# reazon-research/ReazonSpeech

Hardware: NVIDIA H100
Metric: RTFx (audio-s/wall-s) FastConformer-RNNT 619M (higher is better)
Workload: dtype bf16

## Files before the change

reazonspeech_b200/csrc/common.cuh:

```cuda
#pragma once
#include <cuda_bf16.h>
#include <cuda_fp16.h>
#include <cuda_runtime.h>
#include <stdint.h>

#include <atomic>

namespace rs {

struct DeviceOnce {
  std::atomic<unsigned long long> done{0};
  bool pending() const { int d = 0; cudaGetDevice(&d); return ((done.load(std::memory_order_acquire) >> (d & 63)) & 1ull) == 0; }
  void set() { int d = 0; cudaGetDevice(&d); done.fetch_or(1ull << (d & 63), std::memory_order_release); }
};

constexpr int kWarp = 32;

__device__ __forceinline__ uint32_t smem_u32(const void* p) {
  return static_cast<uint32_t>(__cvta_generic_to_shared(p));
}
__device__ __forceinline__ int lane_id() { return threadIdx.x & 31; }
__device__ __forceinline__ int warp_id_uniform() { return __shfl_sync(0xffffffffu, threadIdx.x >> 5, 0); }

__device__ __forceinline__ float warp_sum(float v) {
#pragma unroll
  for (int o = 16; o > 0; o >>= 1) v += __shfl_xor_sync(0xffffffffu, v, o);
  return v;
}
__device__ __forceinline__ float warp_max(float v) {
#pragma unroll
  for (int o = 16; o > 0; o >>= 1) v = fmaxf(v, __shfl_xor_sync(0xffffffffu, v, o));
  return v;
}

__device__ __forceinline__ uint32_t pack_bf16x2(float lo, float hi) {
  __nv_bfloat162 t = __floats2bfloat162_rn(lo, hi);
  return *reinterpret_cast<uint32_t*>(&t);
}
__device__ __forceinline__ uint32_t pack_f16x2(float lo, float hi) {
  __half2 t = __floats2half2_rn(lo, hi);
  return *reinterpret_cast<uint32_t*>(&t);
}
__device__ __forceinline__ float2 unpack_bf16x2(uint32_t v) {
  __nv_bfloat162 t = *reinterpret_cast<__nv_bfloat162*>(&v);
  return __bfloat1622float2(t);
}
__device__ __forceinline__ float bf16_lo(uint32_t v) { return __uint_as_float(v << 16); }
__device__ __forceinline__ float bf16_hi(uint32_t v) { return __uint_as_float(v & 0xffff0000u); }

__device__ __forceinline__ float sigmoidf_fast(float x) {
  float e, r;
  asm("ex2.approx.ftz.f32 %0, %1;" : "=f"(e) : "f"(x * -1.4426950408889634f));
  asm("rcp.approx.ftz.f32 %0, %1;" : "=f"(r) : "f"(1.0f + e));
  return r;
}
__device__ __forceinline__ float sigmoidf_accurate(float x) { return 1.0f / (1.0f + expf(-x)); }
__device__ __forceinline__ float swishf_fast(float x) { return x * sigmoidf_fast(x); }

__device__ __forceinline__ void mbar_init(uint32_t bar, uint32_t count) {
  asm volatile("mbarrier.init.shared::cta.b64 [%0], %1;" ::"r"(bar), "r"(count));
}
__device__ __forceinline__ void fence_barrier_init() {
  asm volatile("fence.mbarrier_init.release.cluster;" ::: "memory");
}
__device__ __forceinline__ void fence_proxy_async() {
  asm volatile("fence.proxy.async.shared::cta;" ::: "memory");
}
__device__ __forceinline__ void mbar_arrive(uint32_t bar) {
  asm volatile("mbarrier.arrive.shared::cta.b64 _, [%0];" ::"r"(bar) : "memory");
}
__device__ __forceinline__ void mbar_arrive_expect_tx(uint32_t bar, uint32_t bytes) {
  asm volatile("mbarrier.arrive.expect_tx.shared::cta.b64 _, [%0], %1;" ::"r"(bar), "r"(bytes) : "memory");
}
__device__ __forceinline__ bool mbar_try_wait(uint32_t bar, uint32_t parity) {
  uint32_t ok;
  asm volatile(
      "{\n\t.reg .pred p;\n\t"
      "mbarrier.try_wait.parity.shared::cta.b64 p, [%1], %2;\n\t"
      "selp.u32 %0, 1, 0, p;\n\t}"
      : "=r"(ok)
      : "r"(bar), "r"(parity)
      : "memory");
  return ok != 0;
}
__device__ __forceinline__ void mbar_wait(uint32_t bar, uint32_t parity) {
  while (!mbar_try_wait(bar, parity)) {
  }
}

__device__ __forceinline__ void tma_prefetch_desc(const void* desc) {
  asm volatile("prefetch.tensormap [%0];" ::"l"(desc) : "memory");
}
__device__ __forceinline__ void tma_load_2d(uint32_t smem_dst, const void* desc, int c0, int c1, uint32_t bar) {
  asm volatile(
      "cp.async.bulk.tensor.2d.shared::cluster.global.tile.mbarrier::complete_tx::bytes [%0], [%1, {%3, %4}], [%2];"
      ::"r"(smem_dst), "l"(desc), "r"(bar), "r"(c0), "r"(c1)
      : "memory");
}

__device__ __forceinline__ void tma_store_2d(const void* desc, uint32_t smem_src, int c0, int c1) {
  asm volatile("cp.async.bulk.tensor.2d.global.shared::cta.bulk_group [%0, {%2, %3}], [%1];"
               ::"l"(desc), "r"(smem_src), "r"(c0), "r"(c1) : "memory");
}
__device__ __forceinline__ void tma_reduce_add_2d(const void* desc, uint32_t smem_src, int c0, int c1) {
  asm volatile("cp.reduce.async.bulk.tensor.2d.global.shared::cta.add.tile.bulk_group [%0, {%2, %3}], [%1];"
               ::"l"(desc), "r"(smem_src), "r"(c0), "r"(c1) : "memory");
}
__device__ __forceinline__ void bulk_commit() { asm volatile("cp.async.bulk.commit_group;" ::: "memory"); }
template <int N>
__device__ __forceinline__ void bulk_wait_read() { asm volatile("cp.async.bulk.wait_group.read %0;" ::"n"(N) : "memory"); }
template <int N>
__device__ __forceinline__ void bulk_wait() { asm volatile("cp.async.bulk.wait_group %0;" ::"n"(N) : "memory"); }

__device__ __forceinline__ void cp_async16(void* smem, const void* gmem) {
  asm volatile("cp.async.cg.shared.global [%0], [%1], 16;" ::"r"(smem_u32(smem)), "l"(gmem) : "memory");
}
__device__ __forceinline__ void cp_async_wait_all() { asm volatile("cp.async.wait_all;" ::: "memory"); }

__device__ __forceinline__ void stmatrix_x4(uint32_t addr, uint32_t r0, uint32_t r1, uint32_t r2, uint32_t r3) {
  asm volatile("stmatrix.sync.aligned.m8n8.x4.shared.b16 [%0], {%1, %2, %3, %4};"
               ::"r"(addr), "r"(r0), "r"(r1), "r"(r2), "r"(r3) : "memory");
}
__device__ __forceinline__ void stmatrix_x4_trans(uint32_t addr, uint32_t r0, uint32_t r1, uint32_t r2, uint32_t r3) {
  asm volatile("stmatrix.sync.aligned.m8n8.x4.trans.shared.b16 [%0], {%1, %2, %3, %4};"
               ::"r"(addr), "r"(r0), "r"(r1), "r"(r2), "r"(r3) : "memory");
}

template <int N>
__device__ __forceinline__ void setmaxnreg_dec() { asm volatile("setmaxnreg.dec.sync.aligned.u32 %0;" ::"n"(N)); }
template <int N>
__device__ __forceinline__ void setmaxnreg_inc() { asm volatile("setmaxnreg.inc.sync.aligned.u32 %0;" ::"n"(N)); }

__device__ __forceinline__ void wgmma_fence() { asm volatile("wgmma.fence.sync.aligned;" ::: "memory"); }
__device__ __forceinline__ void wgmma_commit() { asm volatile("wgmma.commit_group.sync.aligned;" ::: "memory"); }
template <int N>
__device__ __forceinline__ void wgmma_wait() { asm volatile("wgmma.wait_group.sync.aligned %0;" ::"n"(N) : "memory"); }
__device__ __forceinline__ void named_bar_sync(int id, int threads) { asm volatile("bar.sync %0, %1;" ::"r"(id), "r"(threads) : "memory"); }

__device__ __forceinline__ uint64_t wgmma_desc_k_sw128(uint32_t smem_addr) {
  uint64_t d = 0;
  d |= static_cast<uint64_t>((smem_addr & 0x3ffffu) >> 4);
  d |= static_cast<uint64_t>(1) << 16;
  d |= static_cast<uint64_t>(1024 >> 4) << 32;
  d |= static_cast<uint64_t>(1) << 62;
  return d;
}

__device__ __forceinline__ void wgmma_bf16_ss_n32(float (&d)[16], uint64_t desc_a, uint64_t desc_b, uint32_t accumulate) {
  asm volatile(
      "{\n\t.reg .pred p;\n\t"
      "setp.ne.b32 p, %18, 0;\n\t"
      "wgmma.mma_async.sync.aligned.m64n32k16.f32.bf16.bf16 "
      "{%0, %1, %2, %3, %4, %5, %6, %7, %8, %9, %10, %11, %12, %13, %14, %15}, %16, %17, p, 1, 1, 0, 0;\n\t}"
      :
        "+f"(d[0]), "+f"(d[1]), "+f"(d[2]), "+f"(d[3]), "+f"(d[4]), "+f"(d[5]), "+f"(d[6]), "+f"(d[7]),
        "+f"(d[8]), "+f"(d[9]), "+f"(d[10]), "+f"(d[11]), "+f"(d[12]), "+f"(d[13]), "+f"(d[14]), "+f"(d[15])
      : "l"(desc_a), "l"(desc_b), "r"(accumulate));
}

__device__ __forceinline__ void wgmma_bf16_ss_n64(float (&d)[32], uint64_t desc_a, uint64_t desc_b, uint32_t accumulate) {
  asm volatile(
      "{\n\t.reg .pred p;\n\t"
      "setp.ne.b32 p, %34, 0;\n\t"
      "wgmma.mma_async.sync.aligned.m64n64k16.f32.bf16.bf16 "
      "{%0, %1, %2, %3, %4, %5, %6, %7, %8, %9, %10, %11, %12, %13, %14, %15, %16, %17, %18, %19, %20, %21, %22, %23, %24, %25, %26, %27, %28, %29, %30, %31}, %32, %33, p, 1, 1, 0, 0;\n\t}"
      :
        "+f"(d[0]), "+f"(d[1]), "+f"(d[2]), "+f"(d[3]), "+f"(d[4]), "+f"(d[5]), "+f"(d[6]), "+f"(d[7]),
        "+f"(d[8]), "+f"(d[9]), "+f"(d[10]), "+f"(d[11]), "+f"(d[12]), "+f"(d[13]), "+f"(d[14]), "+f"(d[15]),
        "+f"(d[16]), "+f"(d[17]), "+f"(d[18]), "+f"(d[19]), "+f"(d[20]), "+f"(d[21]), "+f"(d[22]), "+f"(d[23]),
        "+f"(d[24]), "+f"(d[25]), "+f"(d[26]), "+f"(d[27]), "+f"(d[28]), "+f"(d[29]), "+f"(d[30]), "+f"(d[31])
      : "l"(desc_a), "l"(desc_b), "r"(accumulate));
}

__device__ __forceinline__ void wgmma_bf16_ss_n128(float (&d)[64], uint64_t desc_a, uint64_t desc_b, uint32_t accumulate) {
  asm volatile(
      "{\n\t.reg .pred p;\n\t"
      "setp.ne.b32 p, %66, 0;\n\t"
      "wgmma.mma_async.sync.aligned.m64n128k16.f32.bf16.bf16 "
      "{%0, %1, %2, %3, %4, %5, %6, %7, %8, %9, %10, %11, %12, %13, %14, %15, %16, %17, %18, %19, %20, %21, %22, %23, %24, %25, %26, %27, %28, %29, %30, %31, %32, %33, %34, %35, %36, %37, %38, %39, %40, %41, %42, %43, %44, %45, %46, %47, %48, %49, %50, %51, %52, %53, %54, %55, %56, %57, %58, %59, %60, %61, %62, %63}, %64, %65, p, 1, 1, 0, 0;\n\t}"
      :
        "+f"(d[0]), "+f"(d[1]), "+f"(d[2]), "+f"(d[3]), "+f"(d[4]), "+f"(d[5]), "+f"(d[6]), "+f"(d[7]),
        "+f"(d[8]), "+f"(d[9]), "+f"(d[10]), "+f"(d[11]), "+f"(d[12]), "+f"(d[13]), "+f"(d[14]), "+f"(d[15]),
        "+f"(d[16]), "+f"(d[17]), "+f"(d[18]), "+f"(d[19]), "+f"(d[20]), "+f"(d[21]), "+f"(d[22]), "+f"(d[23]),
        "+f"(d[24]), "+f"(d[25]), "+f"(d[26]), "+f"(d[27]), "+f"(d[28]), "+f"(d[29]), "+f"(d[30]), "+f"(d[31]),
        "+f"(d[32]), "+f"(d[33]), "+f"(d[34]), "+f"(d[35]), "+f"(d[36]), "+f"(d[37]), "+f"(d[38]), "+f"(d[39]),
        "+f"(d[40]), "+f"(d[41]), "+f"(d[42]), "+f"(d[43]), "+f"(d[44]), "+f"(d[45]), "+f"(d[46]), "+f"(d[47]),
        "+f"(d[48]), "+f"(d[49]), "+f"(d[50]), "+f"(d[51]), "+f"(d[52]), "+f"(d[53]), "+f"(d[54]), "+f"(d[55]),
        "+f"(d[56]), "+f"(d[57]), "+f"(d[58]), "+f"(d[59]), "+f"(d[60]), "+f"(d[61]), "+f"(d[62]), "+f"(d[63])
      : "l"(desc_a), "l"(desc_b), "r"(accumulate));
}

__device__ __forceinline__ void wgmma_bf16_ss_n256(float (&d)[128], uint64_t desc_a, uint64_t desc_b, uint32_t accumulate) {
  asm volatile(
      "{\n\t.reg .pred p;\n\t"
      "setp.ne.b32 p, %130, 0;\n\t"
      "wgmma.mma_async.sync.aligned.m64n256k16.f32.bf16.bf16 "
      "{%0, %1, %2, %3, %4, %5, %6, %7, %8, %9, %10, %11, %12, %13, %14, %15, %16, %17, %18, %19, %20, %21, %22, %23, %24, %25, %26, %27, %28, %29, %30, %31, "
      "%32, %33, %34, %35, %36, %37, %38, %39, %40, %41, %42, %43, %44, %45, %46, %47, %48, %49, %50, %51, %52, %53, %54, %55, %56, %57, %58, %59, %60, %61, %62, %63, "
      "%64, %65, %66, %67, %68, %69, %70, %71, %72, %73, %74, %75, %76, %77, %78, %79, %80, %81, %82, %83, %84, %85, %86, %87, %88, %89, %90, %91, %92, %93, %94, %95, "
      "%96, %97, %98, %99, %100, %101, %102, %103, %104, %105, %106, %107, %108, %109, %110, %111, %112, %113, %114, %115, %116, %117, %118, %119, %120, %121, %122, %123, %124, %125, %126, %127}, "
      "%128, %129, p, 1, 1, 0, 0;\n\t}"
      :
        "+f"(d[0]), "+f"(d[1]), "+f"(d[2]), "+f"(d[3]), "+f"(d[4]), "+f"(d[5]), "+f"(d[6]), "+f"(d[7]),
        "+f"(d[8]), "+f"(d[9]), "+f"(d[10]), "+f"(d[11]), "+f"(d[12]), "+f"(d[13]), "+f"(d[14]), "+f"(d[15]),
        "+f"(d[16]), "+f"(d[17]), "+f"(d[18]), "+f"(d[19]), "+f"(d[20]), "+f"(d[21]), "+f"(d[22]), "+f"(d[23]),
        "+f"(d[24]), "+f"(d[25]), "+f"(d[26]), "+f"(d[27]), "+f"(d[28]), "+f"(d[29]), "+f"(d[30]), "+f"(d[31]),
        "+f"(d[32]), "+f"(d[33]), "+f"(d[34]), "+f"(d[35]), "+f"(d[36]), "+f"(d[37]), "+f"(d[38]), "+f"(d[39]),
        "+f"(d[40]), "+f"(d[41]), "+f"(d[42]), "+f"(d[43]), "+f"(d[44]), "+f"(d[45]), "+f"(d[46]), "+f"(d[47]),
        "+f"(d[48]), "+f"(d[49]), "+f"(d[50]), "+f"(d[51]), "+f"(d[52]), "+f"(d[53]), "+f"(d[54]), "+f"(d[55]),
        "+f"(d[56]), "+f"(d[57]), "+f"(d[58]), "+f"(d[59]), "+f"(d[60]), "+f"(d[61]), "+f"(d[62]), "+f"(d[63]),
        "+f"(d[64]), "+f"(d[65]), "+f"(d[66]), "+f"(d[67]), "+f"(d[68]), "+f"(d[69]), "+f"(d[70]), "+f"(d[71]),
        "+f"(d[72]), "+f"(d[73]), "+f"(d[74]), "+f"(d[75]), "+f"(d[76]), "+f"(d[77]), "+f"(d[78]), "+f"(d[79]),
        "+f"(d[80]), "+f"(d[81]), "+f"(d[82]), "+f"(d[83]), "+f"(d[84]), "+f"(d[85]), "+f"(d[86]), "+f"(d[87]),
        "+f"(d[88]), "+f"(d[89]), "+f"(d[90]), "+f"(d[91]), "+f"(d[92]), "+f"(d[93]), "+f"(d[94]), "+f"(d[95]),
        "+f"(d[96]), "+f"(d[97]), "+f"(d[98]), "+f"(d[99]), "+f"(d[100]), "+f"(d[101]), "+f"(d[102]), "+f"(d[103]),
        "+f"(d[104]), "+f"(d[105]), "+f"(d[106]), "+f"(d[107]), "+f"(d[108]), "+f"(d[109]), "+f"(d[110]), "+f"(d[111]),
        "+f"(d[112]), "+f"(d[113]), "+f"(d[114]), "+f"(d[115]), "+f"(d[116]), "+f"(d[117]), "+f"(d[118]), "+f"(d[119]),
        "+f"(d[120]), "+f"(d[121]), "+f"(d[122]), "+f"(d[123]), "+f"(d[124]), "+f"(d[125]), "+f"(d[126]), "+f"(d[127])
      : "l"(desc_a), "l"(desc_b), "r"(accumulate));
}

__device__ __forceinline__ void wgmma_f16_ss_n64(float (&d)[32], uint64_t desc_a, uint64_t desc_b, uint32_t accumulate) {
  asm volatile(
      "{\n\t.reg .pred p;\n\t"
      "setp.ne.b32 p, %34, 0;\n\t"
      "wgmma.mma_async.sync.aligned.m64n64k16.f32.f16.f16 "
      "{%0, %1, %2, %3, %4, %5, %6, %7, %8, %9, %10, %11, %12, %13, %14, %15, %16, %17, %18, %19, %20, %21, %22, %23, %24, %25, %26, %27, %28, %29, %30, %31}, %32, %33, p, 1, 1, 0, 0;\n\t}"
      :
        "+f"(d[0]), "+f"(d[1]), "+f"(d[2]), "+f"(d[3]), "+f"(d[4]), "+f"(d[5]), "+f"(d[6]), "+f"(d[7]),
        "+f"(d[8]), "+f"(d[9]), "+f"(d[10]), "+f"(d[11]), "+f"(d[12]), "+f"(d[13]), "+f"(d[14]), "+f"(d[15]),
        "+f"(d[16]), "+f"(d[17]), "+f"(d[18]), "+f"(d[19]), "+f"(d[20]), "+f"(d[21]), "+f"(d[22]), "+f"(d[23]),
        "+f"(d[24]), "+f"(d[25]), "+f"(d[26]), "+f"(d[27]), "+f"(d[28]), "+f"(d[29]), "+f"(d[30]), "+f"(d[31])
      : "l"(desc_a), "l"(desc_b), "r"(accumulate));
}

__device__ __forceinline__ void wgmma_bf16_rs_n128(float (&d)[64], const uint32_t (&a)[4], uint64_t desc_b, uint32_t accumulate) {
  asm volatile(
      "{\n\t.reg .pred p;\n\t"
      "setp.ne.b32 p, %69, 0;\n\t"
      "wgmma.mma_async.sync.aligned.m64n128k16.f32.bf16.bf16 "
      "{%0, %1, %2, %3, %4, %5, %6, %7, %8, %9, %10, %11, %12, %13, %14, %15, %16, %17, %18, %19, %20, %21, %22, %23, %24, %25, %26, %27, %28, %29, %30, %31, %32, %33, %34, %35, %36, %37, %38, %39, %40, %41, %42, %43, %44, %45, %46, %47, %48, %49, %50, %51, %52, %53, %54, %55, %56, %57, %58, %59, %60, %61, %62, %63}, {%64, %65, %66, %67}, %68, p, 1, 1, 0;\n\t}"
      :
        "+f"(d[0]), "+f"(d[1]), "+f"(d[2]), "+f"(d[3]), "+f"(d[4]), "+f"(d[5]), "+f"(d[6]), "+f"(d[7]),
        "+f"(d[8]), "+f"(d[9]), "+f"(d[10]), "+f"(d[11]), "+f"(d[12]), "+f"(d[13]), "+f"(d[14]), "+f"(d[15]),
        "+f"(d[16]), "+f"(d[17]), "+f"(d[18]), "+f"(d[19]), "+f"(d[20]), "+f"(d[21]), "+f"(d[22]), "+f"(d[23]),
        "+f"(d[24]), "+f"(d[25]), "+f"(d[26]), "+f"(d[27]), "+f"(d[28]), "+f"(d[29]), "+f"(d[30]), "+f"(d[31]),
        "+f"(d[32]), "+f"(d[33]), "+f"(d[34]), "+f"(d[35]), "+f"(d[36]), "+f"(d[37]), "+f"(d[38]), "+f"(d[39]),
        "+f"(d[40]), "+f"(d[41]), "+f"(d[42]), "+f"(d[43]), "+f"(d[44]), "+f"(d[45]), "+f"(d[46]), "+f"(d[47]),
        "+f"(d[48]), "+f"(d[49]), "+f"(d[50]), "+f"(d[51]), "+f"(d[52]), "+f"(d[53]), "+f"(d[54]), "+f"(d[55]),
        "+f"(d[56]), "+f"(d[57]), "+f"(d[58]), "+f"(d[59]), "+f"(d[60]), "+f"(d[61]), "+f"(d[62]), "+f"(d[63])
      : "r"(a[0]), "r"(a[1]), "r"(a[2]), "r"(a[3]), "l"(desc_b), "r"(accumulate));
}


__device__ __forceinline__ uint4 ldg_nc_v4(const void* p) {
  uint4 r;
  asm volatile("ld.global.nc.L1::no_allocate.v4.u32 {%0, %1, %2, %3}, [%4];" : "=r"(r.x), "=r"(r.y), "=r"(r.z), "=r"(r.w) : "l"(p));
  return r;
}

}
```

reazonspeech_b200/csrc/gemm_wgmma.cu:

```cuda
#include <cuda.h>
#include <cstdio>
#include <cstdlib>
#include <cstring>

#include "../../include/rs_engine.h"
#include "common.cuh"
#include "kernels.h"

namespace rs {

constexpr int BM = 128;
constexpr int BK = 64;
constexpr int kConsumerWarps = 8;
constexpr int kGemmThreads = 128 + 32 * kConsumerWarps;
constexpr int kABytes = BM * BK * 2;
constexpr int kEpiBufs = 3, kEpiBufBytes = 4096;
constexpr int kBiasBytes = 256 * 4;
constexpr int kProducerRegs = 40, kConsumerRegs = 232;

struct GemmDev {
  const float* bias;
  int M, N, K;
  int epilogue;
  float alpha;
  int split;
};
template <int BN>
struct GemmCfg {
  static constexpr int kBBytes = BN * BK * 2;
  static constexpr int kStageBytes = kABytes + kBBytes;
  static constexpr int kEpiBytes = 2 * (kEpiBufs * kEpiBufBytes + kBiasBytes);
  static constexpr int kFixedBytes = 1024  + 256  + kEpiBytes;
  static constexpr int kStages = (227 * 1024 - kFixedBytes) / kStageBytes;
  static constexpr int kSmemBytes = kStages * kStageBytes + kFixedBytes;
  static_assert(2 * 8 * kStages <= 256, "barrier area");
  static_assert(kStageBytes % 1024 == 0, "epilogue buffers need the 1024 B alignment of the 128 B swizzle");
};

__device__ __forceinline__ uint32_t sw64(int row, int chunk) { return static_cast<uint32_t>(row * 64 + ((chunk ^ ((row >> 1) & 3)) << 4)); }

template <int BN, int EG>
__global__ void __launch_bounds__(kGemmThreads, 1)
gemm_bf16_tn_kernel(const __grid_constant__ CUtensorMap tm_a, const __grid_constant__ CUtensorMap tm_b,
                    const __grid_constant__ CUtensorMap tm_out, const __grid_constant__ CUtensorMap tm_out2, const GemmDev p) {
  using Cfg = GemmCfg<BN>;
  extern __shared__ uint8_t smem_raw[];
  const uint32_t smem_base = (smem_u32(smem_raw) + 1023u) & ~1023u;
  const uint32_t epi_base = smem_base + Cfg::kStages * Cfg::kStageBytes;
  const uint32_t bar_base = epi_base + Cfg::kEpiBytes;
  auto full_bar = [&](int s) { return bar_base + 8u * s; };
  auto empty_bar = [&](int s) { return bar_base + 8u * (Cfg::kStages + s); };
  auto smem_a = [&](int s) { return smem_base + s * Cfg::kStageBytes; };
  auto smem_b = [&](int s) { return smem_base + s * Cfg::kStageBytes + kABytes; };
  auto smem_gen = [&](uint32_t addr) { return smem_raw + (addr - smem_u32(smem_raw)); };

  const int warp = warp_id_uniform();
  const int lane = lane_id();
  const int num_m = (p.M + BM - 1) / BM;
  const int num_n = (p.N + BN - 1) / BN;
  const int num_tiles = num_m * num_n;
  const int num_k = p.K / BK;

  if (threadIdx.x == 0) {
    tma_prefetch_desc(&tm_a);
    tma_prefetch_desc(&tm_b);
    tma_prefetch_desc(&tm_out);
    if constexpr (EG == 1) tma_prefetch_desc(&tm_out2);
    for (int s = 0; s < Cfg::kStages; ++s) { mbar_init(full_bar(s), 1); mbar_init(empty_bar(s), kConsumerWarps); }
    fence_barrier_init();
  }
  __syncthreads();

  if (warp < 4) {
    setmaxnreg_dec<kProducerRegs>();
    if (warp == 0 && lane == 0) {
      int stage = 0; uint32_t phase = 0;
      for (int tile = blockIdx.x; tile < num_tiles; tile += gridDim.x) {
        const int m0 = (tile / num_n) * BM, n0 = (tile % num_n) * BN;
        for (int kb = 0; kb < num_k; ++kb) {
          mbar_wait(empty_bar(stage), phase ^ 1u);
          mbar_arrive_expect_tx(full_bar(stage), Cfg::kStageBytes);
          tma_load_2d(smem_a(stage), &tm_a, kb * BK, m0, full_bar(stage));
          tma_load_2d(smem_b(stage), &tm_b, kb * BK, n0, full_bar(stage));
          if (++stage == Cfg::kStages) { stage = 0; phase ^= 1u; }
        }
      }
    }
  } else {
    setmaxnreg_inc<kConsumerRegs>();
    const int cw = warp - 4;
    const int wg = cw >> 2, wq = cw & 3;
    const int rows0 = wg * 64;
    const int tw = threadIdx.x & 127;
    const uint32_t buf0 = epi_base + wg * kEpiBufs * kEpiBufBytes;
    float* bias_s = reinterpret_cast<float*>(smem_gen(epi_base + 2 * kEpiBufs * kEpiBufBytes + wg * kBiasBytes));
    const int g = lane >> 2, t = lane & 3;
    const int mi = lane >> 3, mr = lane & 7;
    int nbuf = 0;
    auto buf = [&]() { return buf0 + nbuf * kEpiBufBytes; };
    auto flush = [&](const CUtensorMap* map, int c0, int c1, bool reduce) {
      fence_proxy_async();
      if (tw == 0) bulk_wait_read<kEpiBufs - 2>();
      named_bar_sync(1 + wg, 128);
      if (tw == 0) {
        if (reduce) tma_reduce_add_2d(map, buf(), c0, c1);
        else tma_store_2d(map, buf(), c0, c1);
        bulk_commit();
      }
      nbuf = nbuf == kEpiBufs - 1 ? 0 : nbuf + 1;
    };

    int stage = 0; uint32_t phase = 0;
    for (int tile = blockIdx.x; tile < num_tiles; tile += gridDim.x) {
      const int m0 = (tile / num_n) * BM, n0 = (tile % num_n) * BN;
      if (4 * tw < min(BN, p.N - n0)) {
        if (p.bias != nullptr) cp_async16(bias_s + 4 * tw, p.bias + n0 + 4 * tw);
        else *reinterpret_cast<float4*>(bias_s + 4 * tw) = make_float4(0.f, 0.f, 0.f, 0.f);
      }
      float d[BN / 2];
      int prev = -1;
      for (int kb = 0; kb < num_k; ++kb) {
        mbar_wait(full_bar(stage), phase);
        const uint64_t da = wgmma_desc_k_sw128(smem_a(stage) + rows0 * 128);
        const uint64_t db = wgmma_desc_k_sw128(smem_b(stage));
        wgmma_fence();
#pragma unroll
        for (int k = 0; k < BK / 16; ++k) {
          if constexpr (BN == 256) wgmma_bf16_ss_n256(d, da + 2u * k, db + 2u * k, (kb | k) != 0 ? 1u : 0u);
          else wgmma_bf16_ss_n64(d, da + 2u * k, db + 2u * k, (kb | k) != 0 ? 1u : 0u);
        }
        wgmma_commit();
        wgmma_wait<1>();
        if (prev >= 0 && lane == 0) mbar_arrive(empty_bar(prev));
        prev = stage;
        if (++stage == Cfg::kStages) { stage = 0; phase ^= 1u; }
      }
      wgmma_wait<0>();
      if (lane == 0) mbar_arrive(empty_bar(prev));
      cp_async_wait_all();
      named_bar_sync(1 + wg, 128);

      const int row_g = m0 + rows0;
#pragma unroll
      for (int c = 0; c < BN / 32; ++c) {
        const int col0 = n0 + c * 32;
        if (col0 < p.N) {
          float v[4][2][2];
#pragma unroll
          for (int j = 0; j < 4; ++j) {
            const float2 b = *reinterpret_cast<const float2*>(bias_s + 32 * c + 8 * j + 2 * t);
#pragma unroll
            for (int h = 0; h < 2; ++h) { v[j][h][0] = d[16 * c + 4 * j + 2 * h] + b.x; v[j][h][1] = d[16 * c + 4 * j + 2 * h + 1] + b.y; }
          }
          const int epi = EG == 1 ? RS_EPI_QKV_VT : p.epilogue;
          if (EG == 1 && col0 >= p.split) {
#pragma unroll
            for (int q = 0; q < 2; ++q) {
              const int dim = 8 * (2 * q + (mi >> 1)) + mr;
              stmatrix_x4_trans(buf() + dim * 128 + (((2 * wq + (mi & 1)) ^ mr) << 4),
                                pack_bf16x2(v[2 * q][0][0], v[2 * q][0][1]), pack_bf16x2(v[2 * q][1][0], v[2 * q][1][1]),
                                pack_bf16x2(v[2 * q + 1][0][0], v[2 * q + 1][0][1]), pack_bf16x2(v[2 * q + 1][1][0], v[2 * q + 1][1][1]));
            }
            flush(&tm_out2, row_g, col0 - p.split, false);
          } else if (epi == RS_EPI_BIAS_GLU_BF16) {
            uint32_t r[2][2];
#pragma unroll
            for (int j = 0; j < 2; ++j)
#pragma unroll
              for (int h = 0; h < 2; ++h)
                r[j][h] = pack_bf16x2(v[j][h][0] * sigmoidf_fast(v[j + 2][h][0]), v[j][h][1] * sigmoidf_fast(v[j + 2][h][1]));
            stmatrix_x4(buf() + sw64(16 * wq + 8 * (mi & 1) + mr, 2 * (c & 1) + (mi >> 1)), r[0][0], r[0][1], r[1][0], r[1][1]);
            if ((c & 1) || col0 + 32 >= p.N) flush(&tm_out, (col0 & ~63) / 2, row_g, false);
          } else if (epi == RS_EPI_BIAS_F32 || epi == RS_EPI_RESID_F32) {
            const bool swp = (g >> 1) & 1;
#pragma unroll
            for (int s = 0; s < 2; ++s) {
#pragma unroll
              for (int k = 0; k < 2; ++k) {
                const int jl = k ^ static_cast<int>(swp);
#pragma unroll
                for (int h = 0; h < 2; ++h) {
                  const int row = 16 * wq + g + 8 * h;
                  const float a0 = jl ? v[2 * s + 1][h][0] : v[2 * s][h][0], a1 = jl ? v[2 * s + 1][h][1] : v[2 * s][h][1];
                  *reinterpret_cast<float2*>(smem_gen(buf() + sw64(row, 2 * jl + (t >> 1)) + 8 * (t & 1))) =
                      make_float2(a0 * p.alpha, a1 * p.alpha);
                }
              }
              flush(&tm_out, col0 + 16 * s, row_g, epi == RS_EPI_RESID_F32);
            }
          } else {
            uint32_t r[4][2];
#pragma unroll
            for (int j = 0; j < 4; ++j)
#pragma unroll
              for (int h = 0; h < 2; ++h) {
                float x0 = v[j][h][0], x1 = v[j][h][1];
                if (epi == RS_EPI_BIAS_RELU_BF16) { x0 = fmaxf(x0, 0.0f); x1 = fmaxf(x1, 0.0f); }
                else if (epi == RS_EPI_BIAS_SWISH_BF16) { x0 = swishf_fast(x0); x1 = swishf_fast(x1); }
                r[j][h] = epi == RS_EPI_BIAS_F16 ? pack_f16x2(x0, x1) : pack_bf16x2(x0, x1);
              }
#pragma unroll
            for (int q = 0; q < 2; ++q)
              stmatrix_x4(buf() + sw64(16 * wq + 8 * (mi & 1) + mr, 2 * q + (mi >> 1)),
                          r[2 * q][0], r[2 * q][1], r[2 * q + 1][0], r[2 * q + 1][1]);
            flush(&tm_out, col0, row_g, false);
          }
        }
      }
    }
    if (tw == 0) bulk_wait<0>();
  }
}

typedef CUresult (*EncodeTiledFn)(CUtensorMap*, CUtensorMapDataType, cuuint32_t, void*, const cuuint64_t*,
                                  const cuuint64_t*, const cuuint32_t*, const cuuint32_t*, CUtensorMapInterleave,
                                  CUtensorMapSwizzle, CUtensorMapL2promotion, CUtensorMapFloatOOBfill);

static EncodeTiledFn get_encode_fn() {
  static EncodeTiledFn fn = nullptr;
  if (fn == nullptr) {
    void* p = nullptr;
    cudaDriverEntryPointQueryResult qres;
    if (cudaGetDriverEntryPoint("cuTensorMapEncodeTiled", &p, cudaEnableDefault, &qres) == cudaSuccess &&
        qres == cudaDriverEntryPointSuccess)
      fn = reinterpret_cast<EncodeTiledFn>(p);
  }
  return fn;
}

static bool make_tmap_2d(CUtensorMap* m, CUtensorMapDataType dtype, int esize, const void* ptr, uint64_t rows, uint64_t cols,
                         uint64_t ld, uint32_t box_cols, uint32_t box_rows, CUtensorMapSwizzle swizzle, char* err) {
  EncodeTiledFn fn = get_encode_fn();
  if (fn == nullptr) { snprintf(err, 256, "cuTensorMapEncodeTiled entry point unavailable"); return false; }
  cuuint64_t dims[2] = {cols, rows};
  cuuint64_t strides[1] = {ld * esize};
  cuuint32_t box[2] = {box_cols, box_rows};
  cuuint32_t estr[2] = {1, 1};
  CUresult r = fn(m, dtype, 2, const_cast<void*>(ptr), dims, strides, box, estr, CU_TENSOR_MAP_INTERLEAVE_NONE, swizzle,
                  CU_TENSOR_MAP_L2_PROMOTION_L2_256B, CU_TENSOR_MAP_FLOAT_OOB_FILL_NONE);
  if (r != CUDA_SUCCESS) { snprintf(err, 256, "cuTensorMapEncodeTiled failed (%d) rows=%llu cols=%llu", (int)r, (unsigned long long)rows, (unsigned long long)cols); return false; }
  return true;
}

bool make_tmap_bf16(CUtensorMap* m, const void* ptr, uint64_t rows, uint64_t cols, uint64_t ld, uint32_t box_rows, char* err) {
  return make_tmap_2d(m, CU_TENSOR_MAP_DATA_TYPE_BFLOAT16, 2, ptr, rows, cols, ld, BK, box_rows, CU_TENSOR_MAP_SWIZZLE_128B, err);
}

inline int epilogue_group(int epilogue) { return epilogue == RS_EPI_QKV_VT ? 1 : 0; }

template <int BN, int EG>
static cudaError_t launch_bn_eg(const GemmArgs& g, int num_sms, cudaStream_t stream, char* err) {
  using Cfg = GemmCfg<BN>;
  static DeviceOnce attr_once;
  if (attr_once.pending()) {
    cudaError_t e = cudaFuncSetAttribute(gemm_bf16_tn_kernel<BN, EG>, cudaFuncAttributeMaxDynamicSharedMemorySize, Cfg::kSmemBytes);
    if (e != cudaSuccess) { snprintf(err, 256, "cudaFuncSetAttribute(smem=%d): %s", Cfg::kSmemBytes, cudaGetErrorString(e)); return e; }
    attr_once.set();
  }
  CUtensorMap tm_a, tm_b, tm_out, tm_out2;
  if (!make_tmap_bf16(&tm_a, g.a, g.M, g.K, g.K, BM, err)) return cudaErrorInvalidValue;
  if (!make_tmap_bf16(&tm_b, g.w, g.N, g.K, g.K, BN, err)) return cudaErrorInvalidValue;
  const bool f32 = g.epilogue == RS_EPI_RESID_F32 || g.epilogue == RS_EPI_BIAS_F32;
  const int ldo = g.epilogue == RS_EPI_BIAS_GLU_BF16 ? g.N / 2 : g.N;
  const CUtensorMapDataType dt = f32 ? CU_TENSOR_MAP_DATA_TYPE_FLOAT32
                                     : g.epilogue == RS_EPI_BIAS_F16 ? CU_TENSOR_MAP_DATA_TYPE_FLOAT16 : CU_TENSOR_MAP_DATA_TYPE_BFLOAT16;
  if (!make_tmap_2d(&tm_out, dt, f32 ? 4 : 2, g.out, g.M, ldo, ldo, f32 ? 16 : 32, 64, CU_TENSOR_MAP_SWIZZLE_64B, err)) return cudaErrorInvalidValue;
  if (EG == 1 && !make_tmap_2d(&tm_out2, CU_TENSOR_MAP_DATA_TYPE_BFLOAT16, 2, g.out2, g.N - g.split, g.M, g.ld2, 64, 32,
                               CU_TENSOR_MAP_SWIZZLE_128B, err))
    return cudaErrorInvalidValue;
  if (EG == 0) tm_out2 = tm_out;
  GemmDev p{g.bias, g.M, g.N, g.K, g.epilogue, g.alpha, g.split};
  const int tiles = ((g.M + BM - 1) / BM) * ((g.N + BN - 1) / BN);
  const int grid = tiles < num_sms ? tiles : num_sms;
  gemm_bf16_tn_kernel<BN, EG><<<grid, kGemmThreads, Cfg::kSmemBytes, stream>>>(tm_a, tm_b, tm_out, tm_out2, p);
  cudaError_t e = cudaGetLastError();
  if (e != cudaSuccess) snprintf(err, 256, "gemm launch (M=%d N=%d K=%d BN=%d): %s", g.M, g.N, g.K, BN, cudaGetErrorString(e));
  return e;
}

template <int BN>
static cudaError_t launch_bn(const GemmArgs& g, int num_sms, cudaStream_t stream, char* err) {
  switch (epilogue_group(g.epilogue)) {
    case 1: return launch_bn_eg<BN, 1>(g, num_sms, stream, err);
    default: return launch_bn_eg<BN, 0>(g, num_sms, stream, err);
  }
}

cudaError_t launch_gemm(const GemmArgs& g, int num_sms, cudaStream_t stream, char* err) {
  if (g.M <= 0 || g.N <= 0 || g.K <= 0 || g.K % BK != 0 || g.N % 32 != 0) {
    snprintf(err, 256, "gemm shape unsupported: M=%d N=%d K=%d (need K%%64==0, N%%32==0)", g.M, g.N, g.K);
    return cudaErrorInvalidValue;
  }
  if ((reinterpret_cast<uintptr_t>(g.a) | reinterpret_cast<uintptr_t>(g.w) | reinterpret_cast<uintptr_t>(g.out) |
       reinterpret_cast<uintptr_t>(g.bias) | reinterpret_cast<uintptr_t>(g.out2)) & 15u) {
    snprintf(err, 256, "gemm operands, bias and outputs must be 16-byte aligned");
    return cudaErrorInvalidValue;
  }
  if (g.epilogue == RS_EPI_RESID_F32 && g.resid == nullptr) { snprintf(err, 256, "gemm: residual epilogue without resid"); return cudaErrorInvalidValue; }
  if (g.epilogue == RS_EPI_QKV_VT && (g.out2 == nullptr || g.split % 32 || g.ld2 % 8 || g.M % 8 || g.ld2 < g.M)) {
    snprintf(err, 256, "gemm: RS_EPI_QKV_VT needs out2, split %% 32 == 0, ld2 %% 8 == 0, M %% 8 == 0, ld2 >= M");
    return cudaErrorInvalidValue;
  }
  if (g.epilogue == RS_EPI_RESID_F32 && g.resid != g.out) {
    cudaError_t e = cudaMemcpyAsync(g.out, g.resid, static_cast<size_t>(g.M) * g.N * sizeof(float), cudaMemcpyDeviceToDevice, stream);
    if (e != cudaSuccess) { snprintf(err, 256, "gemm: residual copy: %s", cudaGetErrorString(e)); return e; }
  }
  if (g.N % 256 == 0 && ((g.M + BM - 1) / BM) * (g.N / 256) >= num_sms) return launch_bn<256>(g, num_sms, stream, err);
  return launch_bn<64>(g, num_sms, stream, err);
}

}
```

Measured before the change: 22440.

## Add ping-pong consumer schedule with BN=128 tiles for costly-epilogue GEMMs

Adds a BN=128 variant of the warp-specialized WGMMA GEMM in which the two consumer warpgroups each own a whole 128-row tile and alternate tiles. A named-barrier turn handoff lets one warpgroup's epilogue overlap the other's mainloop, and the shared stage ring position is recomputed per tile. It is selected only for epilogues with heavy stores (residual f32, bias f32, swish) when K<=1024 and there are at least two tiles per SM. This doubles the accumulator registers per warpgroup and adds barrier handoff complexity in exchange for hiding epilogue cost.

```diff
diff --git a/reazonspeech_b200/csrc/common.cuh b/reazonspeech_b200/csrc/common.cuh
--- a/reazonspeech_b200/csrc/common.cuh
+++ b/reazonspeech_b200/csrc/common.cuh
@@ -136,6 +136,7 @@
 template <int N>
 __device__ __forceinline__ void wgmma_wait() { asm volatile("wgmma.wait_group.sync.aligned %0;" ::"n"(N) : "memory"); }
 __device__ __forceinline__ void named_bar_sync(int id, int threads) { asm volatile("bar.sync %0, %1;" ::"r"(id), "r"(threads) : "memory"); }
+__device__ __forceinline__ void named_bar_arrive(int id, int threads) { asm volatile("bar.arrive %0, %1;" ::"r"(id), "r"(threads) : "memory"); }
 
 __device__ __forceinline__ uint64_t wgmma_desc_k_sw128(uint32_t smem_addr) {
   uint64_t d = 0;
diff --git a/reazonspeech_b200/csrc/gemm_schedule.cuh b/reazonspeech_b200/csrc/gemm_schedule.cuh
--- /dev/null
+++ b/reazonspeech_b200/csrc/gemm_schedule.cuh
@@ -0,0 +1,27 @@
+#pragma once
+#include <stdint.h>
+
+#ifdef __CUDACC__
+#define RS_SCHED_HD __host__ __device__ __forceinline__
+#else
+#define RS_SCHED_HD inline
+#endif
+
+namespace rs {
+
+struct PingPongTurn {
+  bool wait;
+  bool pass;
+};
+
+RS_SCHED_HD PingPongTurn pingpong_turn(int tile, int num_tiles, int grid) {
+  return PingPongTurn{tile >= grid, tile + grid < num_tiles};
+}
+
+RS_SCHED_HD void ring_start(int i, int num_k, int stages, int& stage, uint32_t& phase) {
+  const int q = i * num_k;
+  stage = q % stages;
+  phase = static_cast<uint32_t>(q / stages) & 1u;
+}
+
+}
diff --git a/reazonspeech_b200/csrc/gemm_wgmma.cu b/reazonspeech_b200/csrc/gemm_wgmma.cu
--- a/reazonspeech_b200/csrc/gemm_wgmma.cu
+++ b/reazonspeech_b200/csrc/gemm_wgmma.cu
@@ -5,6 +5,7 @@
 
 #include "../../include/rs_engine.h"
 #include "common.cuh"
+#include "gemm_schedule.cuh"
 #include "kernels.h"
 
 namespace rs {
@@ -16,6 +17,7 @@
 constexpr int kABytes = BM * BK * 2;
 constexpr int kEpiBufs = 3, kEpiBufBytes = 4096;
 constexpr int kBiasBytes = 256 * 4;
+constexpr int kTurnBar = 3;
 constexpr int kProducerRegs = 40, kConsumerRegs = 232;
 
 struct GemmDev {
@@ -27,6 +29,8 @@
 };
 template <int BN>
 struct GemmCfg {
+  static constexpr bool kPingPong = BN == 128;
+  static constexpr int kRowHalves = kPingPong ? 2 : 1;
   static constexpr int kBBytes = BN * BK * 2;
   static constexpr int kStageBytes = kABytes + kBBytes;
   static constexpr int kEpiBytes = 2 * (kEpiBufs * kEpiBufBytes + kBiasBytes);
@@ -66,7 +70,7 @@
     tma_prefetch_desc(&tm_b);
     tma_prefetch_desc(&tm_out);
     if constexpr (EG == 1) tma_prefetch_desc(&tm_out2);
-    for (int s = 0; s < Cfg::kStages; ++s) { mbar_init(full_bar(s), 1); mbar_init(empty_bar(s), kConsumerWarps); }
+    for (int s = 0; s < Cfg::kStages; ++s) { mbar_init(full_bar(s), 1); mbar_init(empty_bar(s), Cfg::kPingPong ? 4 : kConsumerWarps); }
     fence_barrier_init();
   }
   __syncthreads();
@@ -90,7 +94,7 @@
     setmaxnreg_inc<kConsumerRegs>();
     const int cw = warp - 4;
     const int wg = cw >> 2, wq = cw & 3;
-    const int rows0 = wg * 64;
+    const int rows0 = Cfg::kPingPong ? 0 : wg * 64;
     const int tw = threadIdx.x & 127;
     const uint32_t buf0 = epi_base + wg * kEpiBufs * kEpiBufBytes;
     float* bias_s = reinterpret_cast<float*>(smem_gen(epi_base + 2 * kEpiBufs * kEpiBufBytes + wg * kBiasBytes));
@@ -110,24 +114,37 @@
       nbuf = nbuf == kEpiBufs - 1 ? 0 : nbuf + 1;
     };
 
+    constexpr int kH = Cfg::kRowHalves;
+    const int tile0 = blockIdx.x + (Cfg::kPingPong ? wg * gridDim.x : 0);
+    const int tile_step = (Cfg::kPingPong ? 2 : 1) * gridDim.x;
     int stage = 0; uint32_t phase = 0;
-    for (int tile = blockIdx.x; tile < num_tiles; tile += gridDim.x) {
+    for (int tile = tile0; tile < num_tiles; tile += tile_step) {
       const int m0 = (tile / num_n) * BM, n0 = (tile % num_n) * BN;
       if (4 * tw < min(BN, p.N - n0)) {
         if (p.bias != nullptr) cp_async16(bias_s + 4 * tw, p.bias + n0 + 4 * tw);
         else *reinterpret_cast<float4*>(bias_s + 4 * tw) = make_float4(0.f, 0.f, 0.f, 0.f);
       }
-      float d[BN / 2];
+      PingPongTurn turn{false, false};
+      if constexpr (Cfg::kPingPong) {
+        turn = pingpong_turn(tile, num_tiles, gridDim.x);
+        if (turn.wait) named_bar_sync(kTurnBar + wg, 256);
+        ring_start((tile - blockIdx.x) / gridDim.x, num_k, Cfg::kStages, stage, phase);
+      }
+      float d[kH][BN / 2];
       int prev = -1;
       for (int kb = 0; kb < num_k; ++kb) {
         mbar_wait(full_bar(stage), phase);
-        const uint64_t da = wgmma_desc_k_sw128(smem_a(stage) + rows0 * 128);
         const uint64_t db = wgmma_desc_k_sw128(smem_b(stage));
         wgmma_fence();
 #pragma unroll
         for (int k = 0; k < BK / 16; ++k) {
-          if constexpr (BN == 256) wgmma_bf16_ss_n256(d, da + 2u * k, db + 2u * k, (kb | k) != 0 ? 1u : 0u);
-          else wgmma_bf16_ss_n64(d, da + 2u * k, db + 2u * k, (kb | k) != 0 ? 1u : 0u);
+#pragma unroll
+          for (int h = 0; h < kH; ++h) {
+            const uint64_t da = wgmma_desc_k_sw128(smem_a(stage) + (rows0 + 64 * h) * 128);
+            if constexpr (BN == 256) wgmma_bf16_ss_n256(d[h], da + 2u * k, db + 2u * k, (kb | k) != 0 ? 1u : 0u);
+            else if constexpr (BN == 128) wgmma_bf16_ss_n128(d[h], da + 2u * k, db + 2u * k, (kb | k) != 0 ? 1u : 0u);
+            else wgmma_bf16_ss_n64(d[h], da + 2u * k, db + 2u * k, (kb | k) != 0 ? 1u : 0u);
+          }
         }
         wgmma_commit();
         wgmma_wait<1>();
@@ -135,14 +152,16 @@
         prev = stage;
         if (++stage == Cfg::kStages) { stage = 0; phase ^= 1u; }
       }
+      if (turn.pass) named_bar_arrive(kTurnBar + (wg ^ 1), 256);
       wgmma_wait<0>();
       if (lane == 0) mbar_arrive(empty_bar(prev));
       cp_async_wait_all();
       named_bar_sync(1 + wg, 128);
 
-      const int row_g = m0 + rows0;
-#pragma unroll
-      for (int c = 0; c < BN / 32; ++c) {
+#pragma unroll
+      for (int e = 0; e < kH * (BN / 32); ++e) {
+        const int mh = e / (BN / 32), c = e % (BN / 32);
+        const int row_g = m0 + rows0 + 64 * mh;
         const int col0 = n0 + c * 32;
         if (col0 < p.N) {
           float v[4][2][2];
@@ -150,7 +169,7 @@
           for (int j = 0; j < 4; ++j) {
             const float2 b = *reinterpret_cast<const float2*>(bias_s + 32 * c + 8 * j + 2 * t);
 #pragma unroll
-            for (int h = 0; h < 2; ++h) { v[j][h][0] = d[16 * c + 4 * j + 2 * h] + b.x; v[j][h][1] = d[16 * c + 4 * j + 2 * h + 1] + b.y; }
+            for (int h = 0; h < 2; ++h) { v[j][h][0] = d[mh][16 * c + 4 * j + 2 * h] + b.x; v[j][h][1] = d[mh][16 * c + 4 * j + 2 * h + 1] + b.y; }
           }
           const int epi = EG == 1 ? RS_EPI_QKV_VT : p.epilogue;
           if (EG == 1 && col0 >= p.split) {
@@ -280,10 +299,9 @@
 
 template <int BN>
 static cudaError_t launch_bn(const GemmArgs& g, int num_sms, cudaStream_t stream, char* err) {
-  switch (epilogue_group(g.epilogue)) {
-    case 1: return launch_bn_eg<BN, 1>(g, num_sms, stream, err);
-    default: return launch_bn_eg<BN, 0>(g, num_sms, stream, err);
-  }
+  if constexpr (BN != 128)
+    if (epilogue_group(g.epilogue) == 1) return launch_bn_eg<BN, 1>(g, num_sms, stream, err);
+  return launch_bn_eg<BN, 0>(g, num_sms, stream, err);
 }
 
 cudaError_t launch_gemm(const GemmArgs& g, int num_sms, cudaStream_t stream, char* err) {
@@ -305,6 +323,9 @@
     cudaError_t e = cudaMemcpyAsync(g.out, g.resid, static_cast<size_t>(g.M) * g.N * sizeof(float), cudaMemcpyDeviceToDevice, stream);
     if (e != cudaSuccess) { snprintf(err, 256, "gemm: residual copy: %s", cudaGetErrorString(e)); return e; }
   }
+  const bool costly_epilogue = g.epilogue == RS_EPI_RESID_F32 || g.epilogue == RS_EPI_BIAS_F32 || g.epilogue == RS_EPI_BIAS_SWISH_BF16;
+  if (costly_epilogue && g.K <= 1024 && g.N % 128 == 0 && ((g.M + BM - 1) / BM) * (g.N / 128) >= 2 * num_sms)
+    return launch_bn<128>(g, num_sms, stream, err);
   if (g.N % 256 == 0 && ((g.M + BM - 1) / BM) * (g.N / 256) >= num_sms) return launch_bn<256>(g, num_sms, stream, err);
   return launch_bn<64>(g, num_sms, stream, err);
 }
```

Result: faster. 22890, median of 6 (+2.0%).

## Ping-pong consumer warpgroups over full-M tile shares to overlap epilogue with MMA

Applied to the files above, without the earlier changes.

Restructures the persistent WGMMA GEMM so each consumer warpgroup computes a whole 128-row by up-to-128-column share, issuing two m64 WGMMAs, instead of both warpgroups splitting one tile by rows. The warpgroups alternate shares and hand off via named barriers, so one group's epilogue overlaps the other's mainloop. The producer loads B in share-sized boxes, and empty barriers now expect half as many arrivals. This doubles accumulator registers per thread and adds cross-warpgroup ordering, which risks register pressure and stalls.

```diff
diff --git a/reazonspeech_b200/csrc/common.cuh b/reazonspeech_b200/csrc/common.cuh
--- a/reazonspeech_b200/csrc/common.cuh
+++ b/reazonspeech_b200/csrc/common.cuh
@@ -136,6 +136,7 @@
 template <int N>
 __device__ __forceinline__ void wgmma_wait() { asm volatile("wgmma.wait_group.sync.aligned %0;" ::"n"(N) : "memory"); }
 __device__ __forceinline__ void named_bar_sync(int id, int threads) { asm volatile("bar.sync %0, %1;" ::"r"(id), "r"(threads) : "memory"); }
+__device__ __forceinline__ void named_bar_arrive(int id, int threads) { asm volatile("bar.arrive %0, %1;" ::"r"(id), "r"(threads) : "memory"); }
 
 __device__ __forceinline__ uint64_t wgmma_desc_k_sw128(uint32_t smem_addr) {
   uint64_t d = 0;
diff --git a/reazonspeech_b200/csrc/gemm_wgmma.cu b/reazonspeech_b200/csrc/gemm_wgmma.cu
--- a/reazonspeech_b200/csrc/gemm_wgmma.cu
+++ b/reazonspeech_b200/csrc/gemm_wgmma.cu
@@ -13,7 +13,7 @@
 constexpr int BK = 64;
 constexpr int kConsumerWarps = 8;
 constexpr int kGemmThreads = 128 + 32 * kConsumerWarps;
-constexpr int kABytes = BM * BK * 2;
+constexpr int kTurnBar = 3;
 constexpr int kEpiBufs = 3, kEpiBufBytes = 4096;
 constexpr int kBiasBytes = 256 * 4;
 constexpr int kProducerRegs = 40, kConsumerRegs = 232;
@@ -27,7 +27,10 @@
 };
 template <int BN>
 struct GemmCfg {
-  static constexpr int kBBytes = BN * BK * 2;
+  static constexpr int kShareCols = BN < 128 ? BN : 128;
+  static constexpr int kShares = BN / kShareCols;
+  static constexpr int kABytes = BM * BK * 2;
+  static constexpr int kBBytes = kShareCols * BK * 2;
   static constexpr int kStageBytes = kABytes + kBBytes;
   static constexpr int kEpiBytes = 2 * (kEpiBufs * kEpiBufBytes + kBiasBytes);
   static constexpr int kFixedBytes = 1024  + 256  + kEpiBytes;
@@ -51,7 +54,7 @@
   auto full_bar = [&](int s) { return bar_base + 8u * s; };
   auto empty_bar = [&](int s) { return bar_base + 8u * (Cfg::kStages + s); };
   auto smem_a = [&](int s) { return smem_base + s * Cfg::kStageBytes; };
-  auto smem_b = [&](int s) { return smem_base + s * Cfg::kStageBytes + kABytes; };
+  auto smem_b = [&](int s) { return smem_base + s * Cfg::kStageBytes + Cfg::kABytes; };
   auto smem_gen = [&](uint32_t addr) { return smem_raw + (addr - smem_u32(smem_raw)); };
 
   const int warp = warp_id_uniform();
@@ -66,7 +69,7 @@
     tma_prefetch_desc(&tm_b);
     tma_prefetch_desc(&tm_out);
     if constexpr (EG == 1) tma_prefetch_desc(&tm_out2);
-    for (int s = 0; s < Cfg::kStages; ++s) { mbar_init(full_bar(s), 1); mbar_init(empty_bar(s), kConsumerWarps); }
+    for (int s = 0; s < Cfg::kStages; ++s) { mbar_init(full_bar(s), 1); mbar_init(empty_bar(s), kConsumerWarps / 2); }
     fence_barrier_init();
   }
   __syncthreads();
@@ -77,12 +80,14 @@
       int stage = 0; uint32_t phase = 0;
       for (int tile = blockIdx.x; tile < num_tiles; tile += gridDim.x) {
         const int m0 = (tile / num_n) * BM, n0 = (tile % num_n) * BN;
-        for (int kb = 0; kb < num_k; ++kb) {
-          mbar_wait(empty_bar(stage), phase ^ 1u);
-          mbar_arrive_expect_tx(full_bar(stage), Cfg::kStageBytes);
-          tma_load_2d(smem_a(stage), &tm_a, kb * BK, m0, full_bar(stage));
-          tma_load_2d(smem_b(stage), &tm_b, kb * BK, n0, full_bar(stage));
-          if (++stage == Cfg::kStages) { stage = 0; phase ^= 1u; }
+        for (int h = 0; h < Cfg::kShares; ++h) {
+          for (int kb = 0; kb < num_k; ++kb) {
+            mbar_wait(empty_bar(stage), phase ^ 1u);
+            mbar_arrive_expect_tx(full_bar(stage), Cfg::kStageBytes);
+            tma_load_2d(smem_a(stage), &tm_a, kb * BK, m0, full_bar(stage));
+            tma_load_2d(smem_b(stage), &tm_b, kb * BK, n0 + h * Cfg::kShareCols, full_bar(stage));
+            if (++stage == Cfg::kStages) { stage = 0; phase ^= 1u; }
+          }
         }
       }
     }
@@ -90,7 +95,6 @@
     setmaxnreg_inc<kConsumerRegs>();
     const int cw = warp - 4;
     const int wg = cw >> 2, wq = cw & 3;
-    const int rows0 = wg * 64;
     const int tw = threadIdx.x & 127;
     const uint32_t buf0 = epi_base + wg * kEpiBufs * kEpiBufBytes;
     float* bias_s = reinterpret_cast<float*>(smem_gen(epi_base + 2 * kEpiBufs * kEpiBufBytes + wg * kBiasBytes));
@@ -110,103 +114,122 @@
       nbuf = nbuf == kEpiBufs - 1 ? 0 : nbuf + 1;
     };
 
+    const int num_units = (num_tiles - 1 - static_cast<int>(blockIdx.x)) / static_cast<int>(gridDim.x) + 1;
+    const int num_shares = num_units * Cfg::kShares;
     int stage = 0; uint32_t phase = 0;
-    for (int tile = blockIdx.x; tile < num_tiles; tile += gridDim.x) {
-      const int m0 = (tile / num_n) * BM, n0 = (tile % num_n) * BN;
-      if (4 * tw < min(BN, p.N - n0)) {
+    auto advance = [&](int n) { stage += n; phase ^= static_cast<uint32_t>(stage / Cfg::kStages) & 1u; stage %= Cfg::kStages; };
+    advance(wg * num_k);
+    for (int sh = wg; sh < num_shares; sh += 2) {
+      const int tile = blockIdx.x + (sh / Cfg::kShares) * gridDim.x;
+      const int m0 = (tile / num_n) * BM, n0 = (tile % num_n) * BN + (sh % Cfg::kShares) * Cfg::kShareCols;
+      if (4 * tw < min(Cfg::kShareCols, p.N - n0)) {
         if (p.bias != nullptr) cp_async16(bias_s + 4 * tw, p.bias + n0 + 4 * tw);
         else *reinterpret_cast<float4*>(bias_s + 4 * tw) = make_float4(0.f, 0.f, 0.f, 0.f);
       }
-      float d[BN / 2];
+      if (sh > 0) named_bar_sync(kTurnBar + wg, 256);
+      const bool pass_turn = sh + 1 < num_shares;
+      float d0[Cfg::kShareCols / 2], d1[Cfg::kShareCols / 2];
       int prev = -1;
       for (int kb = 0; kb < num_k; ++kb) {
         mbar_wait(full_bar(stage), phase);
-        const uint64_t da = wgmma_desc_k_sw128(smem_a(stage) + rows0 * 128);
+        const uint64_t da = wgmma_desc_k_sw128(smem_a(stage));
         const uint64_t db = wgmma_desc_k_sw128(smem_b(stage));
         wgmma_fence();
 #pragma unroll
         for (int k = 0; k < BK / 16; ++k) {
-          if constexpr (BN == 256) wgmma_bf16_ss_n256(d, da + 2u * k, db + 2u * k, (kb | k) != 0 ? 1u : 0u);
-          else wgmma_bf16_ss_n64(d, da + 2u * k, db + 2u * k, (kb | k) != 0 ? 1u : 0u);
+          const uint32_t acc = (kb | k) != 0 ? 1u : 0u;
+          if constexpr (Cfg::kShareCols == 128) {
+            wgmma_bf16_ss_n128(d0, da + 2u * k, db + 2u * k, acc);
+            wgmma_bf16_ss_n128(d1, da + 512u + 2u * k, db + 2u * k, acc);
+          } else {
+            wgmma_bf16_ss_n64(d0, da + 2u * k, db + 2u * k, acc);
+            wgmma_bf16_ss_n64(d1, da + 512u + 2u * k, db + 2u * k, acc);
+          }
         }
         wgmma_commit();
+        if (kb == num_k - 1 && pass_turn) named_bar_arrive(kTurnBar + (wg ^ 1), 256);
         wgmma_wait<1>();
         if (prev >= 0 && lane == 0) mbar_arrive(empty_bar(prev));
         prev = stage;
         if (++stage == Cfg::kStages) { stage = 0; phase ^= 1u; }
       }
+      advance(num_k);
       wgmma_wait<0>();
       if (lane == 0) mbar_arrive(empty_bar(prev));
       cp_async_wait_all();
       named_bar_sync(1 + wg, 128);
 
-      const int row_g = m0 + rows0;
-#pragma unroll
-      for (int c = 0; c < BN / 32; ++c) {
-        const int col0 = n0 + c * 32;
-        if (col0 < p.N) {
-          float v[4][2][2];
-#pragma unroll
-          for (int j = 0; j < 4; ++j) {
-            const float2 b = *reinterpret_cast<const float2*>(bias_s + 32 * c + 8 * j + 2 * t);
-#pragma unroll
-            for (int h = 0; h < 2; ++h) { v[j][h][0] = d[16 * c + 4 * j + 2 * h] + b.x; v[j][h][1] = d[16 * c + 4 * j + 2 * h + 1] + b.y; }
-          }
-          const int epi = EG == 1 ? RS_EPI_QKV_VT : p.epilogue;
-          if (EG == 1 && col0 >= p.split) {
-#pragma unroll
-            for (int q = 0; q < 2; ++q) {
-              const int dim = 8 * (2 * q + (mi >> 1)) + mr;
-              stmatrix_x4_trans(buf() + dim * 128 + (((2 * wq + (mi & 1)) ^ mr) << 4),
-                                pack_bf16x2(v[2 * q][0][0], v[2 * q][0][1]), pack_bf16x2(v[2 * q][1][0], v[2 * q][1][1]),
-                                pack_bf16x2(v[2 * q + 1][0][0], v[2 * q + 1][0][1]), pack_bf16x2(v[2 * q + 1][1][0], v[2 * q + 1][1][1]));
+      auto epilogue_block = [&](const auto& d, int mh) {
+        const int row_g = m0 + 64 * mh;
+#pragma unroll
+        for (int c = 0; c < Cfg::kShareCols / 32; ++c) {
+          const int col0 = n0 + c * 32;
+          if (col0 < p.N) {
+            float v[4][2][2];
+#pragma unroll
+            for (int j = 0; j < 4; ++j) {
+              const float2 b = *reinterpret_cast<const float2*>(bias_s + 32 * c + 8 * j + 2 * t);
+#pragma unroll
+              for (int h = 0; h < 2; ++h) { v[j][h][0] = d[16 * c + 4 * j + 2 * h] + b.x; v[j][h][1] = d[16 * c + 4 * j + 2 * h + 1] + b.y; }
             }
-            flush(&tm_out2, row_g, col0 - p.split, false);
-          } else if (epi == RS_EPI_BIAS_GLU_BF16) {
-            uint32_t r[2][2];
-#pragma unroll
-            for (int j = 0; j < 2; ++j)
-#pragma unroll
-              for (int h = 0; h < 2; ++h)
-                r[j][h] = pack_bf16x2(v[j][h][0] * sigmoidf_fast(v[j + 2][h][0]), v[j][h][1] * sigmoidf_fast(v[j + 2][h][1]));
-            stmatrix_x4(buf() + sw64(16 * wq + 8 * (mi & 1) + mr, 2 * (c & 1) + (mi >> 1)), r[0][0], r[0][1], r[1][0], r[1][1]);
-            if ((c & 1) || col0 + 32 >= p.N) flush(&tm_out, (col0 & ~63) / 2, row_g, false);
-          } else if (epi == RS_EPI_BIAS_F32 || epi == RS_EPI_RESID_F32) {
-            const bool swp = (g >> 1) & 1;
-#pragma unroll
-            for (int s = 0; s < 2; ++s) {
-#pragma unroll
-              for (int k = 0; k < 2; ++k) {
-                const int jl = k ^ static_cast<int>(swp);
+            const int epi = EG == 1 ? RS_EPI_QKV_VT : p.epilogue;
+            if (EG == 1 && col0 >= p.split) {
+#pragma unroll
+              for (int q = 0; q < 2; ++q) {
+                const int dim = 8 * (2 * q + (mi >> 1)) + mr;
+                stmatrix_x4_trans(buf() + dim * 128 + (((2 * wq + (mi & 1)) ^ mr) << 4),
+                                  pack_bf16x2(v[2 * q][0][0], v[2 * q][0][1]), pack_bf16x2(v[2 * q][1][0], v[2 * q][1][1]),
+                                  pack_bf16x2(v[2 * q + 1][0][0], v[2 * q + 1][0][1]), pack_bf16x2(v[2 * q + 1][1][0], v[2 * q + 1][1][1]));
+              }
+              flush(&tm_out2, row_g, col0 - p.split, false);
+            } else if (epi == RS_EPI_BIAS_GLU_BF16) {
+              uint32_t r[2][2];
+#pragma unroll
+              for (int j = 0; j < 2; ++j)
+#pragma unroll
+                for (int h = 0; h < 2; ++h)
+                  r[j][h] = pack_bf16x2(v[j][h][0] * sigmoidf_fast(v[j + 2][h][0]), v[j][h][1] * sigmoidf_fast(v[j + 2][h][1]));
+              stmatrix_x4(buf() + sw64(16 * wq + 8 * (mi & 1) + mr, 2 * (c & 1) + (mi >> 1)), r[0][0], r[0][1], r[1][0], r[1][1]);
+              if ((c & 1) || col0 + 32 >= p.N) flush(&tm_out, (col0 & ~63) / 2, row_g, false);
+            } else if (epi == RS_EPI_BIAS_F32 || epi == RS_EPI_RESID_F32) {
+              const bool swp = (g >> 1) & 1;
+#pragma unroll
+              for (int s = 0; s < 2; ++s) {
+#pragma unroll
+                for (int k = 0; k < 2; ++k) {
+                  const int jl = k ^ static_cast<int>(swp);
+#pragma unroll
+                  for (int h = 0; h < 2; ++h) {
+                    const int row = 16 * wq + g + 8 * h;
+                    const float a0 = jl ? v[2 * s + 1][h][0] : v[2 * s][h][0], a1 = jl ? v[2 * s + 1][h][1] : v[2 * s][h][1];
+                    *reinterpret_cast<float2*>(smem_gen(buf() + sw64(row, 2 * jl + (t >> 1)) + 8 * (t & 1))) =
+                        make_float2(a0 * p.alpha, a1 * p.alpha);
+                  }
+                }
+                flush(&tm_out, col0 + 16 * s, row_g, epi == RS_EPI_RESID_F32);
+              }
+            } else {
+              uint32_t r[4][2];
+#pragma unroll
+              for (int j = 0; j < 4; ++j)
 #pragma unroll
                 for (int h = 0; h < 2; ++h) {
-                  const int row = 16 * wq + g + 8 * h;
-                  const float a0 = jl ? v[2 * s + 1][h][0] : v[2 * s][h][0], a1 = jl ? v[2 * s + 1][h][1] : v[2 * s][h][1];
-                  *reinterpret_cast<float2*>(smem_gen(buf() + sw64(row, 2 * jl + (t >> 1)) + 8 * (t & 1))) =
-                      make_float2(a0 * p.alpha, a1 * p.alpha);
+                  float x0 = v[j][h][0], x1 = v[j][h][1];
+                  if (epi == RS_EPI_BIAS_RELU_BF16) { x0 = fmaxf(x0, 0.0f); x1 = fmaxf(x1, 0.0f); }
+                  else if (epi == RS_EPI_BIAS_SWISH_BF16) { x0 = swishf_fast(x0); x1 = swishf_fast(x1); }
+                  r[j][h] = epi == RS_EPI_BIAS_F16 ? pack_f16x2(x0, x1) : pack_bf16x2(x0, x1);
                 }
-              }
-              flush(&tm_out, col0 + 16 * s, row_g, epi == RS_EPI_RESID_F32);
+#pragma unroll
+              for (int q = 0; q < 2; ++q)
+                stmatrix_x4(buf() + sw64(16 * wq + 8 * (mi & 1) + mr, 2 * q + (mi >> 1)),
+                            r[2 * q][0], r[2 * q][1], r[2 * q + 1][0], r[2 * q + 1][1]);
+              flush(&tm_out, col0, row_g, false);
             }
-          } else {
-            uint32_t r[4][2];
-#pragma unroll
-            for (int j = 0; j < 4; ++j)
-#pragma unroll
-              for (int h = 0; h < 2; ++h) {
-                float x0 = v[j][h][0], x1 = v[j][h][1];
-                if (epi == RS_EPI_BIAS_RELU_BF16) { x0 = fmaxf(x0, 0.0f); x1 = fmaxf(x1, 0.0f); }
-                else if (epi == RS_EPI_BIAS_SWISH_BF16) { x0 = swishf_fast(x0); x1 = swishf_fast(x1); }
-                r[j][h] = epi == RS_EPI_BIAS_F16 ? pack_f16x2(x0, x1) : pack_bf16x2(x0, x1);
-              }
-#pragma unroll
-            for (int q = 0; q < 2; ++q)
-              stmatrix_x4(buf() + sw64(16 * wq + 8 * (mi & 1) + mr, 2 * q + (mi >> 1)),
-                          r[2 * q][0], r[2 * q][1], r[2 * q + 1][0], r[2 * q + 1][1]);
-            flush(&tm_out, col0, row_g, false);
           }
         }
-      }
+      };
+      epilogue_block(d0, 0);
+      epilogue_block(d1, 1);
     }
     if (tw == 0) bulk_wait<0>();
   }
@@ -259,7 +282,7 @@
   }
   CUtensorMap tm_a, tm_b, tm_out, tm_out2;
   if (!make_tmap_bf16(&tm_a, g.a, g.M, g.K, g.K, BM, err)) return cudaErrorInvalidValue;
-  if (!make_tmap_bf16(&tm_b, g.w, g.N, g.K, g.K, BN, err)) return cudaErrorInvalidValue;
+  if (!make_tmap_bf16(&tm_b, g.w, g.N, g.K, g.K, Cfg::kShareCols, err)) return cudaErrorInvalidValue;
   const bool f32 = g.epilogue == RS_EPI_RESID_F32 || g.epilogue == RS_EPI_BIAS_F32;
   const int ldo = g.epilogue == RS_EPI_BIAS_GLU_BF16 ? g.N / 2 : g.N;
   const CUtensorMapDataType dt = f32 ? CU_TENSOR_MAP_DATA_TYPE_FLOAT32
```

Measured after the change: 22410 before, 22660 after, median of 6. +1.1%, better.
